# mpeg5/xevd

Measured on AMD Instinct MI355X. Metric: frames/sec (bit-exact YUV) + achieved HBM GB/s, higher is better.
Workload: dtype s16; 1 GPU; cfg4_main_8k_10b_ra; width=7680, height=4320, bit_depth=10, batches_resident=4, residual_pass_ahead=True, parallelism=1 stream on 1 GPU

## Files before the change

xevd_amd/csrc/itdq_body.h:

```cpp
#pragma once
#include "xgpu_internal.h"

typedef short v2s __attribute__((ext_vector_type(2)));

static __constant__ uint32_t k_tmp[2730];
__host__ __device__ constexpr int tmp_base(int log2n) { return log2n == 1 ? 0 : log2n == 2 ? 2 : log2n == 3 ? 10 : log2n == 4 ? 42 : log2n == 5 ? 170 : 682; }

static __constant__ uint32_t k_atsp[2][680];
__host__ __device__ constexpr int atsp_base(int log2n) { return log2n == 2 ? 0 : log2n == 3 ? 8 : log2n == 4 ? 40 : 168; }

static void upload_transform_tables_tu(const int *tm, const int16_t *ats, hipStream_t s)
{
    static uint32_t apk[2][680];
    for (int t = 0; t < 2; t++) {
        int src = 0;
        for (int l = 2; l <= 5; l++) {
            const int N = 1 << l, dst = atsp_base(l);
            for (int k2 = 0; k2 < N / 2; k2++)
                for (int n = 0; n < N; n++)
                    apk[t][dst + k2 * N + n] = (uint32_t)(uint16_t)ats[t * 1360 + src + (2 * k2) * N + n] |
                                               ((uint32_t)(uint16_t)ats[t * 1360 + src + (2 * k2 + 1) * N + n] << 16);
            src += N * N;
        }
    }
    (void)hipMemcpyToSymbolAsync(HIP_SYMBOL(k_atsp), apk, sizeof(apk), 0, hipMemcpyHostToDevice, s);
    static uint32_t packed[2730];
    int src = 0;
    for (int l = 1; l <= 6; l++) {
        const int N = 1 << l, dst = tmp_base(l);
        for (int k2 = 0; k2 < N / 2; k2++)
            for (int n = 0; n < N; n++)
                packed[dst + k2 * N + n] = (uint32_t)(uint16_t)(int16_t)tm[src + (2 * k2) * N + n] |
                                           ((uint32_t)(uint16_t)(int16_t)tm[src + (2 * k2 + 1) * N + n] << 16);
        src += N * N;
    }
    (void)hipMemcpyToSymbolAsync(HIP_SYMBOL(k_tmp), packed, sizeof(packed), 0, hipMemcpyHostToDevice, s);
    (void)hipStreamSynchronize(s);
}

__device__ __forceinline__ int clip16(int v) { return min(max(v, -32768), 32767); }
__device__ __forceinline__ int dot2(uint32_t a, uint32_t b, int c)
{
    return __builtin_amdgcn_sdot2(__builtin_bit_cast(v2s, a), __builtin_bit_cast(v2s, b), c, false);
}

__host__ __device__ constexpr int itdq_group(int lw, int lh)
{
    const int W = 1 << lw, H = 1 << lh;
    const int l1 = W * (H > 16 ? H / 16 : 1), l2 = H * (W > 16 ? W / 16 : 1);
    return 256 / (l1 > l2 ? l1 : l2);
}

#define ITDQ_PLANES_DWORDS 4608
#define ITDQ_LDS_DWORDS (ITDQ_PLANES_DWORDS + 2048)
#define ITDQ_MAX_G 128

__device__ __forceinline__ uint32_t wave_or(uint32_t v)
{
#pragma unroll
    for (int m = 32; m >= 1; m >>= 1) v |= (uint32_t)__shfl_xor((int)v, m, 64);
    return v;
}

template <int LW, int LH, bool IQT>
__device__ __forceinline__ void itdq_item(const ItdqArgs &a, const TbWave wv, uint32_t *lds, uint32_t *s_rm, uint32_t *s_cm)
{
    constexpr int W = 1 << LW, H = 1 << LH;
    constexpr int N1 = H > 16 ? 16 : H, C1 = H / N1;
    constexpr int N2 = W > 16 ? 16 : W, C2 = W / N2;
    constexpr int G = itdq_group(LW, LH);
    constexpr int RS = W / 2 + 1;
    constexpr int PLANE = G * H * RS;
    constexpr bool UNI1 = (G * W) % 64 == 0, UNI2 = (G * H) % 64 == 0;
    static_assert(2 * PLANE <= ITDQ_PLANES_DWORDS && G * W * H <= 4096 && G <= ITDQ_MAX_G, "LDS budget");
    constexpr int PLANES_DWORDS = IQT ? ITDQ_PLANES_DWORDS / 2 : ITDQ_PLANES_DWORDS;
    constexpr bool RMASK = H >= 16, CMASK = W >= 16;
    const int t = threadIdx.x;
    if (RMASK || CMASK) {
        if (t < G) { s_rm[t] = 0; s_cm[t] = 0; }
        __syncthreads();
    }
    const uint32_t *tmh = (wv.tr_v == TR_DCT2 || LH < 2 || LH > 5) ? k_tmp + tmp_base(LH) : k_atsp[wv.tr_v - 1] + atsp_base(LH);
    const uint32_t *tmw = (wv.tr_h == TR_DCT2 || LW < 2 || LW > 5) ? k_tmp + tmp_base(LW) : k_atsp[wv.tr_h - 1] + atsp_base(LW);
    const bool s16_mid = IQT || wv.tr_v != TR_DCT2 || wv.tr_h != TR_DCT2;
    int16_t *ldsh = (int16_t *)lds;
    int16_t *ldsl = (int16_t *)(lds + PLANE);
    uint32_t *ldsc = lds + PLANES_DWORDS;

    {
        constexpr int S = W * H, UN = S >= 8 ? 8 : 4;
        constexpr int odd = (LW + LH) & 1;
        const int shift = 20 - 14 - (15 - a.bd - ((LW + LH) >> 1)) + (odd ? 8 : 0);
        const long long offset = shift == 0 ? 0 : 1ll << (shift - 1);
        for (int u = t; u < G * S / UN; u += 256) {
            const int p = (u * UN) / S, o = (u * UN) % S;
            if (p >= wv.count) break;
            const TbRec tb = a.tbs[wv.first + p];
            const int qp = tb.qp, sidx = qp % 6;
            const int sbase = sidx == 0 ? 40 : sidx == 1 ? 45 : sidx == 2 ? 51 : sidx == 3 ? 57 : sidx == 4 ? 64 : (IQT ? 72 : 71);
            const long long mul = (long long)(sbase << (qp / 6)) * (odd ? 181 : 1);
            const int16_t *src = a.coef + tb.off + ((o >> LW) << tb.log2s) + (o & (W - 1));
            uint32_t raw[UN / 2];
            if constexpr (UN == 8) { const uint4 v = *(const uint4 *)src; raw[0] = v.x; raw[1] = v.y; raw[2] = v.z; raw[3] = v.w; }
            else { const uint2 v = *(const uint2 *)src; raw[0] = v.x; raw[1] = v.y; }
#pragma unroll
            for (int i = 0; i < UN / 2; i++) {
                if (raw[i] == 0) continue;
                const int c0 = (int16_t)(raw[i] & 0xFFFF), c1 = (int16_t)(raw[i] >> 16);
                const long long l0 = ((long long)c0 * mul + offset) >> shift, l1 = ((long long)c1 * mul + offset) >> shift;
                const int v0 = (int)min(max(l0, -32768ll), 32767ll), v1 = (int)min(max(l1, -32768ll), 32767ll);
                raw[i] = (uint32_t)(uint16_t)v0 | ((uint32_t)(uint16_t)v1 << 16);
                if (RMASK) atomicOr(&s_rm[p], 1u << ((o + 2 * i) >> (LW + 1)));
                if (CMASK) atomicOr(&s_cm[p], 1u << (((o + 2 * i) & (W - 1)) >> 1));
            }
#pragma unroll
            for (int i = 0; i < UN / 2; i++) ldsc[(p * S + o) / 2 + i] = raw[i];
        }
    }
    __syncthreads();

    uint32_t rows1 = 0;
    if (RMASK) {
        const int p1 = (t % (G * W)) >> LW;
        rows1 = (uint32_t)__builtin_amdgcn_readfirstlane((int)wave_or((t < G * W * C1 && p1 < wv.count) ? s_rm[p1] : 0u));
    }
    if (t < G * W * C1) {
        const int idx = t % (G * W);
        int chunk = t / (G * W);
        if (UNI1) chunk = __builtin_amdgcn_readfirstlane(chunk);
        const int p = idx >> LW, j = idx & (W - 1);
        const bool valid = p < wv.count;
        const int16_t *src = (const int16_t *)ldsc + p * (W * H) + j;

        int acc[N1];
#pragma unroll
        for (int n = 0; n < N1; n++) acc[n] = 0;
        if (RMASK) {
            for (uint32_t m = rows1; m; m &= m - 1) {
                const int k2 = __builtin_ctz(m);
                const uint32_t vp = valid ? ((uint32_t)(uint16_t)src[(2 * k2) * W] | ((uint32_t)(uint16_t)src[(2 * k2 + 1) * W] << 16)) : 0u;
                const uint32_t *row = tmh + k2 * H + chunk * N1;
#pragma unroll
                for (int n = 0; n < N1; n++) acc[n] = dot2(row[n], vp, acc[n]);
            }
        } else {
            for (int k2 = 0; k2 < H / 2; k2++) {
                const uint32_t vp = valid ? ((uint32_t)(uint16_t)src[(2 * k2) * W] | ((uint32_t)(uint16_t)src[(2 * k2 + 1) * W] << 16)) : 0u;
                if (__ballot(vp != 0) == 0) continue;
                const uint32_t *row = tmh + k2 * H + chunk * N1;
#pragma unroll
                for (int n = 0; n < N1; n++) acc[n] = dot2(row[n], vp, acc[n]);
            }
        }
        const int base = (p * H + chunk * N1) * (2 * RS) + j;
        if (CMASK && !(valid && ((s_cm[p] >> (j >> 1)) & 1))) {
        } else if (s16_mid) {
#pragma unroll
            for (int n = 0; n < N1; n++) ldsh[base + n * (2 * RS)] = (int16_t)clip16((acc[n] + 64) >> 7);
        } else {
#pragma unroll
            for (int n = 0; n < N1; n++) {
                ldsh[base + n * (2 * RS)] = (int16_t)(acc[n] >> 15);
                ldsl[base + n * (2 * RS)] = (int16_t)(acc[n] & 0x7FFF);
            }
        }
    }
    __syncthreads();

    uint32_t cols2 = 0;
    if (CMASK) {
        const int p2 = (t % (G * H)) >> LH;
        cols2 = (uint32_t)__builtin_amdgcn_readfirstlane((int)wave_or((t < G * H * C2 && p2 < wv.count) ? s_cm[p2] : 0u));
    }
    if (t < G * H * C2) {
        const int idx = t % (G * H);
        int chunk = t / (G * H);
        if (UNI2) chunk = __builtin_amdgcn_readfirstlane(chunk);
        const int p = idx >> LH, r = idx & (H - 1);
        if (p >= wv.count) return;
        const uint32_t own = CMASK ? s_cm[p] : 0xFFFFFFFFu;
        const TbRec tb = a.tbs[wv.first + p];
        const int shift2 = s16_mid ? 12 - (a.bd - 8) : 7 + 12 - (a.bd - 8);
        const uint32_t *inh = lds + (p * H + r) * RS;
        const uint32_t *inl = inh + PLANE;
        int res[N2];
        if (s16_mid) {
            int s[N2];
#pragma unroll
            for (int n = 0; n < N2; n++) s[n] = 1 << (shift2 - 1);
            if (CMASK) {
                for (uint32_t m = cols2; m; m &= m - 1) {
                    const int k2 = __builtin_ctz(m);
                    const uint32_t vp = ((own >> k2) & 1) ? inh[k2] : 0u;
                    const uint32_t *row = tmw + k2 * W + chunk * N2;
#pragma unroll
                    for (int n = 0; n < N2; n++) s[n] = dot2(row[n], vp, s[n]);
                }
            } else {
                for (int k2 = 0; k2 < W / 2; k2++) {
                    const uint32_t vp = inh[k2];
                    if (__ballot(vp != 0) == 0) continue;
                    const uint32_t *row = tmw + k2 * W + chunk * N2;
#pragma unroll
                    for (int n = 0; n < N2; n++) s[n] = dot2(row[n], vp, s[n]);
                }
            }
#pragma unroll
            for (int n = 0; n < N2; n++) res[n] = clip16(s[n] >> shift2);
        } else {
            int sh[N2], sl[N2];
#pragma unroll
            for (int n = 0; n < N2; n++) { sh[n] = 0; sl[n] = 0; }
            if (CMASK) {
                for (uint32_t m = cols2; m; m &= m - 1) {
                    const int k2 = __builtin_ctz(m);
                    const bool mine = (own >> k2) & 1;
                    const uint32_t vh = mine ? inh[k2] : 0u, vl = mine ? inl[k2] : 0u;
                    const uint32_t *row = tmw + k2 * W + chunk * N2;
#pragma unroll
                    for (int n = 0; n < N2; n++) { sh[n] = dot2(row[n], vh, sh[n]); sl[n] = dot2(row[n], vl, sl[n]); }
                }
            } else {
                for (int k2 = 0; k2 < W / 2; k2++) {
                    const uint32_t vh = inh[k2], vl = inl[k2];
                    if (__ballot((vh | vl) != 0) == 0) continue;
                    const uint32_t *row = tmw + k2 * W + chunk * N2;
#pragma unroll
                    for (int n = 0; n < N2; n++) { sh[n] = dot2(row[n], vh, sh[n]); sl[n] = dot2(row[n], vl, sl[n]); }
                }
            }
            const long long add = 1ll << (shift2 - 1);
#pragma unroll
            for (int n = 0; n < N2; n++) {
                const long long s = (long long)sh[n] * 32768 + sl[n] + add;
                res[n] = (int)min(max(s >> shift2, -32768ll), 32767ll);
            }
        }
        int16_t *out = a.resid + tb.off + (r << tb.log2s) + chunk * N2;
        if constexpr (N2 >= 8) {
#pragma unroll
            for (int n = 0; n < N2; n += 8) {
                uint4 v;
                v.x = (uint32_t)(uint16_t)res[n + 0] | ((uint32_t)(uint16_t)res[n + 1] << 16);
                v.y = (uint32_t)(uint16_t)res[n + 2] | ((uint32_t)(uint16_t)res[n + 3] << 16);
                v.z = (uint32_t)(uint16_t)res[n + 4] | ((uint32_t)(uint16_t)res[n + 5] << 16);
                v.w = (uint32_t)(uint16_t)res[n + 6] | ((uint32_t)(uint16_t)res[n + 7] << 16);
                *(uint4 *)(out + n) = v;
            }
        } else if constexpr (N2 == 4) {
            uint2 v;
            v.x = (uint32_t)(uint16_t)res[0] | ((uint32_t)(uint16_t)res[1] << 16);
            v.y = (uint32_t)(uint16_t)res[2] | ((uint32_t)(uint16_t)res[3] << 16);
            *(uint2 *)out = v;
        } else {
            *(uint32_t *)out = (uint32_t)(uint16_t)res[0] | ((uint32_t)(uint16_t)res[1] << 16);
        }
    }
}

template <bool IQT>
__device__ __forceinline__ void itdq_dispatch(const ItdqArgs &a, int wi, uint32_t *lds, uint32_t *s_rm, uint32_t *s_cm)
{
    const TbWave wv = a.waves[wi];
#define CASE(lw, lh) case (lw) * 8 + (lh): itdq_item<lw, lh, IQT>(a, wv, lds, s_rm, s_cm); break;
#define ROW(lw) CASE(lw, 1) CASE(lw, 2) CASE(lw, 3) CASE(lw, 4) CASE(lw, 5) CASE(lw, 6)
    switch (wv.log2w * 8 + wv.log2h) {
        ROW(1) ROW(2) ROW(3) ROW(4) ROW(5) ROW(6)
        default: break;
    }
#undef ROW
#undef CASE
}
```

xevd_amd/csrc/k_intra.hip:

```cpp
#include "xgpu_internal.h"
#include "itdq_body.h"

#include <type_traits>
#include "intra_pred.h"

#define INTRA_WAVES 8


__constant__ uint8_t k_htdf_tbl[5][16] = {
    { 0, 0, 2,  6, 10, 14, 19, 23, 28, 32,  36,  41,  45,  49,  53,  57 },
    { 0, 0, 5, 12, 20, 29, 38, 47, 56, 65,  73,  82,  90,  98, 107, 115 },
    { 0, 0, 1,  4,  9, 16, 24, 32, 41, 50,  59,  68,  77,  86,  94, 103 },
    { 0, 0, 3,  9, 19, 32, 47, 64, 81, 99, 117, 135, 154, 179, 205, 230 },
    { 0, 0, 0,  2,  6, 11, 18, 27, 38, 51,  64,  96, 128, 160, 192, 224 },
};
#define HTDF_EXT (66 * 66)

template <bool HTDF> struct IntraLds { static constexpr int WAVE = (HTDF && HTDF_EXT > 3 * NB_LEN) ? HTDF_EXT : 3 * NB_LEN; };

#ifdef INTRA_PROFILE
__device__ uint32_t g_intra_prof[8 * 64];
#define ISTAMP(k) do { if (DEP && t == 0 && item >= INTRA_PROFILE && item < INTRA_PROFILE + 64) g_intra_prof[8 * (item - INTRA_PROFILE) + (k)] = (uint32_t)clock64(); } while (0)
#else
#define ISTAMP(k)
// ... 315 lines not shown
                        for (int q = 0; q < 4; q++) pl[r][q] = vl[nb_sel(md, r, q, 3)];
                if (md == mode_c)
#pragma unroll
                    for (int c = 0; c < 2; c++)
#pragma unroll
                        for (int r = 0; r < 2; r++)
#pragma unroll
                            for (int q = 0; q < 2; q++) pc[c][r][q] = vc[c][nb_sel(md, r, q, 1)];
            }
            }
            int16_t *dy = a.cur_y + y * a.s_l + x;
            uint32_t ol[4][2], oc[2][2];
#pragma unroll
            for (int r = 0; r < 4; r++) {
                ol[r][0] = pack2i(pl[r][0], pl[r][1]); ol[r][1] = pack2i(pl[r][2], pl[r][3]);
                ol[r][0] = recon2i(ol[r][0], (cbf & 1) ? rl_cur[r].x : 0u, maxv); ol[r][1] = recon2i(ol[r][1], (cbf & 1) ? rl_cur[r].y : 0u, maxv);
            }
#pragma unroll
            for (int c = 1; c < 3; c++)
#pragma unroll
                for (int r = 0; r < 2; r++) {
                    oc[c - 1][r] = pack2i(pc[c - 1][r][0], pc[c - 1][r][1]);
                    oc[c - 1][r] = recon2i(oc[c - 1][r], ((cbf >> c) & 1) ? rc_cur[c - 1][r] : 0u, maxv);
                }
            const int coff = (y >> 1) * a.s_c + (x >> 1);
            if (!(nflags & 32u))
#pragma unroll
            for (int r = 0; r < 4; r++) {
                if (DEP) st_coherent2(dy + r * a.s_l, ol[r][0], ol[r][1]); else *(uint2 *)(dy + r * a.s_l) = make_uint2(ol[r][0], ol[r][1]);
            }
            if (!(nflags & 64u))
#pragma unroll
            for (int c = 1; c < 3; c++) {
                int16_t *d = (c == 1 ? a.cur_u : a.cur_v) + coff;
#pragma unroll
                for (int r = 0; r < 2; r++)
                    if (DEP) st_coherent(d + r * a.s_c, oc[c - 1][r]); else *(uint32_t *)(d + r * a.s_c) = oc[c - 1][r];
            }
        }
        if (HTDF && htdf_cu) {
            const uint32_t av = (nflags >> 8) & 0x1FF;
            const bool cmask = (nflags >> 4) & 1;
            const int tidx = (nflags >> 20) & 7;
            const int thr_log2 = tidx == 0 ? 6 : (tidx < 3 ? 7 : 8), shift = thr_log2 - 4, rnd = (1 << shift) >> 1, thr = (1 << thr_log2) - (1 << shift);
            int16_t *tb = s_nb[wv];
            wave_lds_sync();
            const int we = cw + 2, he = chh + 2;
            int16_t *org = a.cur_y + cu_y * a.s_l + cu_x;
            asm volatile("s_waitcnt vmcnt(0)" ::: "memory");
            auto ldw = [&](const int16_t *p) -> uint32_t { return DEP ? ld_coherent(p) : *(const uint32_t *)p; };
            auto ldr = [&](const int16_t *p) -> uint32_t { return ldw((const int16_t *)((uintptr_t)p & ~(uintptr_t)3)); };
            auto pick = [&](const int16_t *p, uint32_t d) -> int16_t { return (int16_t)(((uintptr_t)p & 2) ? d >> 16 : d & 0xFFFFu); };
            const int16_t *p_l = nullptr, *p_r = nullptr, *p_u = nullptr, *p_d = nullptr, *p_c = nullptr;
            uint32_t d_l = 0, d_r = 0, d_u = 0, d_d = 0, d_c = 0;
            if (t < chh) {
                const bool ok_l = ((av >> 1) & 1) && (!cmask || ((avail_le_raw >> (t >> 2)) & 1));
                const bool ok_r = ((av >> 3) & 1) && (!cmask || ((avail_ri >> (t >> 2)) & 1));
                p_l = org + t * a.s_l + (ok_l ? -1 : 0); p_r = org + t * a.s_l + (ok_r ? cw : cw - 1);
                d_l = ldr(p_l); d_r = ldr(p_r);
            }
            if (t < cw) {
                const bool ok_u = (av & 1) && (!cmask || ((avail_up >> (t >> 2)) & 1));
                p_u = org + t - (ok_u ? a.s_l : 0); p_d = org + (chh - 1) * a.s_l + t;
                d_u = ldr(p_u); d_d = ldr(p_d);
            }
            if (t < 4) {
                p_c = t == 0 ? (((av >> 5) & 1) ? org - 1 - a.s_l : org) : t == 1 ? (((av >> 6) & 1) ? org + cw - a.s_l : org + cw - 1)
                    : t == 2 ? (((av >> 7) & 1) ? org - 1 + chh * a.s_l : org + (chh - 1) * a.s_l) : (((av >> 8) & 1) ? org + cw + chh * a.s_l : org + cw - 1 + (chh - 1) * a.s_l);
                d_c = ldr(p_c);
            }
            const int n2 = (cw >> 1) * chh;
            ISTAMP(6);
            for (int i0 = 0; i0 < n2; i0 += 64 * 8) {
                uint32_t d[8];
#pragma unroll
                for (int q = 0; q < 8; q++) {
                    const int i = i0 + q * 64 + t;
                    d[q] = 0;
                    if (i < n2) d[q] = ldw(org + (i >> (lw - 1)) * a.s_l + ((i & ((cw >> 1) - 1)) << 1));
                }
#pragma unroll
                for (int q = 0; q < 8; q++) {
                    const int i = i0 + q * 64 + t, r = i >> (lw - 1), c = (i & ((cw >> 1) - 1)) << 1;
                    if (i < n2) { tb[(r + 1) * we + c + 1] = (int16_t)(d[q] & 0xFFFF); tb[(r + 1) * we + c + 2] = (int16_t)(d[q] >> 16); }
                }
            }
            asm volatile("" : "+v"(d_l), "+v"(d_r), "+v"(d_u), "+v"(d_d), "+v"(d_c));
            if (t < chh) { tb[(t + 1) * we] = pick(p_l, d_l); tb[(t + 1) * we + we - 1] = pick(p_r, d_r); }
            if (t < cw) { tb[t + 1] = pick(p_u, d_u); tb[(he - 1) * we + t + 1] = pick(p_d, d_d); }
            if (t < 4) tb[t == 0 ? 0 : t == 1 ? we - 1 : t == 2 ? we * (he - 1) : we - 1 + we * (he - 1)] = pick(p_c, d_c);
            wave_lds_sync();
            ISTAMP(7);
            const uint32_t *tb32 = (const uint32_t *)k_htdf_tbl[tidx];
            const uint32_t tq0 = uni(tb32[0]), tq1 = uni(tb32[1]), tq2 = uni(tb32[2]), tq3 = uni(tb32[3]);
            auto lutf = [&](int z) -> int {
                const int ab = z < 0 ? -z : z;
                const uint32_t idx = (uint32_t)(((ab + rnd) & thr) >> shift), sel = (idx & 7u) | 0x0C0C0C00u;
                const int e = (int)((idx & 8u) ? __builtin_amdgcn_perm(tq3, tq2, sel) : __builtin_amdgcn_perm(tq1, tq0, sel));
                const int v = ab < thr ? e : ab;
                return z < 0 ? -v : v;
            };
            auto filter_tiles = [&](auto TRc, auto TCc) {
                constexpr int TR = decltype(TRc)::value, TC = decltype(TCc)::value, LR = TR == 4 ? 2 : 1, LC = TC == 4 ? 2 : 1;
                const int tiles_x = cw >> LC, ltx = lw - LC;
                for (int i = t; i < tiles_x * (chh >> LR); i += 64) {
                    const int r = (i >> ltx) << LR, c = (i & (tiles_x - 1)) << LC;
                    int p[TR + 2][TC + 2];
#pragma unroll
                    for (int rr = 0; rr < TR + 2; rr++)
#pragma unroll
                        for (int cc = 0; cc < TC + 2; cc += 2) {
                            const uint32_t d = *(const uint32_t *)&tb[(r + rr) * we + c + cc];
                            p[rr][cc] = (int)(int16_t)(d & 0xFFFF); p[rr][cc + 1] = (int)(int16_t)(d >> 16);
                        }
                    int acc[TR][TC];
#pragma unroll
                    for (int dr = 0; dr < TR; dr++)
#pragma unroll
                        for (int dc = 0; dc < TC; dc++) acc[dr][dc] = 0;
#pragma unroll
                    for (int wr = 0; wr < TR + 1; wr++)
#pragma unroll
                        for (int wc = 0; wc < TC + 1; wc++) {
                            const int x0 = p[wr][wc], x1 = p[wr][wc + 1], x2 = p[wr + 1][wc], x3 = p[wr + 1][wc + 1];
                            const int y0 = x0 + x2, y1 = x1 + x3, y2 = x0 - x2, y3 = x1 - x3;
                            const int z0 = y0 + y1, z1 = lutf(y0 - y1), z2 = lutf(y2 + y3), z3 = lutf(y2 - y3);
                            const int i0_ = z0 + z2, i1_ = z1 + z3, i2_ = z0 - z2, i3_ = z1 - z3;
#pragma unroll
                            for (int row = 0; row < 2; row++)
#pragma unroll
                                for (int col = 0; col < 2; col++) {
                                    const int dr = wr - 1 + row, dc = wc - 1 + col;
                                    if (dr < 0 || dr >= TR || dc < 0 || dc >= TC) continue;
                                    const int v = row == 1 ? (col == 0 ? i2_ + i3_ : i2_ - i3_) : (col == 0 ? i0_ + i1_ : i0_ - i1_);
                                    acc[dr][dc] += v >> 2;
                                }
                        }
#pragma unroll
                    for (int dr = 0; dr < TR; dr++)
#pragma unroll
                        for (int dc = 0; dc < TC; dc += 2) {
                            const int o0 = clip3i(0, maxv, ((int)(int16_t)acc[dr][dc] + 2) >> 2), o1 = clip3i(0, maxv, ((int)(int16_t)acc[dr][dc + 1] + 2) >> 2);
                            if (DEP) st_coherent(org + (r + dr) * a.s_l + c + dc, pack2i(o0, o1)); else *(uint32_t *)(org + (r + dr) * a.s_l + c + dc) = pack2i(o0, o1);
                        }
                }
            };
            if (cw * chh >= 1024) filter_tiles(std::integral_constant<int, 4>{}, std::integral_constant<int, 4>{});
            else                 filter_tiles(std::integral_constant<int, 2>{}, std::integral_constant<int, 2>{});
        }
        ISTAMP(4);
        if (DEP) {
            asm volatile("s_waitcnt vmcnt(0)" ::: "memory");
            ISTAMP(5);
            if (t == 0) __hip_atomic_store(&a.done[item], a.epoch, __ATOMIC_RELAXED, __HIP_MEMORY_SCOPE_AGENT);
        }
        wave_lds_sync();
        if (!DEP) break;
        item = uni(q0.x);
        if (item == 0xFFFFFFFFu) break;
    }
}

#define SB_C0 71
#define SB_UR 144
#define SB_LEN (SB_UR + 72)
#define SMALL_GROUPS (4 * INTRA_WAVES)
__device__ __forceinline__ void intra_small_body(const IntraArgs &a, uint32_t block, int16_t *s_nb_)
{
    int16_t (*s_nb)[3][SB_LEN] = (int16_t (*)[3][SB_LEN])s_nb_;
    const int g = threadIdx.x >> 4, t = threadIdx.x & 15;
    const uint32_t k = block * SMALL_GROUPS + (uint32_t)g;
    if (k >= (uint32_t)a.n_small) return;
    const uint32_t item = (uint32_t)(a.first + a.count - a.n_small) + k;
    int16_t (*nb)[SB_LEN] = s_nb[g];
    const int mid = 1 << (a.bd_l - 1), maxv = (1 << a.bd_l) - 1;
    const uint4 *rec = (const uint4 *)&a.list[item];
    const uint4 q0 = rec[0], q1 = rec[1], q2 = rec[2];
    const uint32_t nflags = q0.y, avail_ul = nflags & 1;
    const int lrf = (int)((nflags >> 23) & 3);
    const uint64_t avail_up = (uint64_t)q0.z | ((lrf & 2) ? 0ull : (uint64_t)q0.w << 32);
    const uint64_t avail_le = (uint64_t)q1.x | ((uint64_t)q1.y << 32);
    const uint32_t gg = q2.x, m = q2.y, ipm = q2.z, coef_off = q2.w;
    const int cu_x = gg & 0xFFFF, cu_y = gg >> 16;
    const int lw = m & 0xFF, lh = (m >> 8) & 0xFF, cbf = (m >> 16) & 0xFF;
    const int mode_l = ipm & 0xFF, mode_c = (ipm >> 8) & 0xFF;
    const int cw = 1 << lw, chh = 1 << lh, scuw = cw >> 2, nscu = scuw * (chh >> 2), cwc = cw >> 1;
    const uint32_t off_u = coef_off + ((cbf & 1) ? (uint32_t)(cw * chh) : 0u);
    const uint32_t off_v = off_u + ((cbf & 2) ? (uint32_t)(cwc * (chh >> 1)) : 0u);
    const bool has = t < nscu;
    const int lx = (t & (scuw - 1)) << 2, ly = (t >> (lw - 2)) << 2;

    uint2 rl[4] = { { 0, 0 }, { 0, 0 }, { 0, 0 }, { 0, 0 } };
    uint32_t rc[2][2] = { { 0, 0 }, { 0, 0 } };
    if (has) {
        if (cbf & 1)
#pragma unroll
            for (int r = 0; r < 4; r++) rl[r] = *(const uint2 *)(a.resid + coef_off + (ly + r) * cw + lx);
#pragma unroll
        for (int c = 1; c < 3; c++)
            if ((cbf >> c) & 1)
#pragma unroll
                for (int r = 0; r < 2; r++) rc[c - 1][r] = *(const uint32_t *)(a.resid + (c == 1 ? off_u : off_v) + ((ly >> 1) + r) * cwc + (lx >> 1));
    }

#pragma unroll
    for (int c = 0; c < 3; c++) {
        const int16_t *plane = c == 0 ? a.cur_y : (c == 1 ? a.cur_u : a.cur_v);
        const int s = c ? a.s_c : a.s_l, sh = c ? 1 : 0, ush = c ? 1 : 2;
        const int16_t *org = plane + (cu_y >> sh) * s + (cu_x >> sh);
        const int n = (cw + chh) >> sh;
        const int eu = min(2 * t, n - 2), e0 = min(t, n - 1), e1 = min(t + 16, n - 1);
        const uint32_t vu = *(const uint32_t *)(org - s + eu);
        const uint32_t v0 = (uint16_t)org[e0 * s - 1], v1 = (uint16_t)org[e1 * s - 1], vc = (uint16_t)org[-s - 1];
        const uint32_t midp = (uint32_t)mid * 0x10001u;
        if (2 * t < n) *(uint32_t *)&nb[c][SB_C0 + 1 + 2 * t] = ((avail_up >> (eu >> ush)) & 1) ? vu : midp;
        if (t < n) nb[c][SB_C0 - 1 - t] = (int16_t)(((avail_le >> (e0 >> ush)) & 1) ? v0 : (uint32_t)mid);
        if (t + 16 < n) nb[c][SB_C0 - 1 - (t + 16)] = (int16_t)(((avail_le >> (e1 >> ush)) & 1) ? v1 : (uint32_t)mid);
        if (t == 0) nb[c][SB_C0] = (int16_t)(avail_ul ? vc : (uint32_t)mid);
        if (n > 32) {
            for (int e = 2 * t + 32; e < n; e += 32)
                *(uint32_t *)&nb[c][SB_C0 + 1 + e] = ((avail_up >> (e >> ush)) & 1) ? *(const uint32_t *)(org - s + e) : midp;
            for (int e = t + 32; e < n; e += 16)
                nb[c][SB_C0 - 1 - e] = ((avail_le >> (e >> ush)) & 1) ? org[e * s - 1] : (int16_t)mid;
        }
    }
    wave_lds_sync();
#pragma unroll
    for (int c = 0; c < 3; c++) {
        const int mode = c ? mode_c : mode_l;
        const int w = c ? cw >> 1 : cw, h = c ? chh >> 1 : chh;
        if (mode == 0) {
            int acc = 0;
            for (int e = t; e < w + h; e += 16) acc += e < h ? nb[c][SB_C0 - 1 - e] : nb[c][SB_C0 + 1 + e - h];
            acc = row_sum16(acc);
            if (t == 0) nb[c][NB_DC] = (int16_t)((acc + w) >> ((c ? lw - 1 : lw) + 1));
        } else if (mode == 4) {
            for (int e = t; e < w + h; e += 16) nb[c][SB_UR + e] = (int16_t)((nb[c][SB_C0 + 1 + e] + nb[c][SB_C0 - 1 - e]) >> 1);
        }
    }
    wave_lds_sync();
    if (!has) return;
    const int x = cu_x + lx, y = cu_y + ly;
    int pl[4][4], pc[2][2][2];
    int vl[7], vc[2][3];
    nb_fetch<7, SB_C0, SB_UR>(nb[0], mode_l, lx, ly, vl);
    nb_fetch<3, SB_C0, SB_UR>(nb[1], mode_c, lx >> 1, ly >> 1, vc[0]);
    nb_fetch<3, SB_C0, SB_UR>(nb[2], mode_c, lx >> 1, ly >> 1, vc[1]);
#pragma unroll
    for (int md = 0; md < 5; md++) {
        if (md == mode_l)
#pragma unroll
            for (int r = 0; r < 4; r++)
#pragma unroll
                for (int q = 0; q < 4; q++) pl[r][q] = vl[nb_sel(md, r, q, 3)];
        if (md == mode_c)
#pragma unroll
            for (int c = 0; c < 2; c++)
#pragma unroll
                for (int r = 0; r < 2; r++)
#pragma unroll
                    for (int q = 0; q < 2; q++) pc[c][r][q] = vc[c][nb_sel(md, r, q, 1)];
    }
    int16_t *dy = a.cur_y + y * a.s_l + x;
    const int coff = (y >> 1) * a.s_c + (x >> 1);
    if (!(nflags & 32u))
#pragma unroll
        for (int r = 0; r < 4; r++) {
            const uint32_t o0 = recon2i(pack2i(pl[r][0], pl[r][1]), (cbf & 1) ? rl[r].x : 0u, maxv), o1 = recon2i(pack2i(pl[r][2], pl[r][3]), (cbf & 1) ? rl[r].y : 0u, maxv);
            *(uint2 *)(dy + r * a.s_l) = make_uint2(o0, o1);
        }
    if (!(nflags & 64u))
#pragma unroll
        for (int c = 1; c < 3; c++) {
            int16_t *d = (c == 1 ? a.cur_u : a.cur_v) + coff;
#pragma unroll
            for (int r = 0; r < 2; r++)
                *(uint32_t *)(d + r * a.s_c) = recon2i(pack2i(pc[c - 1][r][0], pc[c - 1][r][1]), ((cbf >> c) & 1) ? rc[c - 1][r] : 0u, maxv);
        }
}

__global__ __launch_bounds__(64 * INTRA_WAVES) void k_intra_l1(const IntraArgs a, uint32_t big)
{
    constexpr int BIG_LDS = INTRA_WAVES * IntraLds<false>::WAVE, SMALL_LDS = SMALL_GROUPS * 3 * SB_LEN;
    __shared__ __attribute__((aligned(16))) int16_t s_nb[BIG_LDS > SMALL_LDS ? BIG_LDS : SMALL_LDS];
    if (blockIdx.x < big) {
        IntraArgs b = a;
        b.count = a.count - a.n_small;
        intra_body<false, 0, false, false, INTRA_WAVES>(b, blockIdx.x, s_nb, nullptr);
    } else intra_small_body(a, blockIdx.x - big, s_nb);
}

template <bool DEP, int EIPD, bool IBC, bool HTDF>
__global__ __launch_bounds__(64 * INTRA_WAVES) void k_intra(const IntraArgs a)
{
    __shared__ __attribute__((aligned(16))) int16_t s_nb[INTRA_WAVES * IntraLds<HTDF>::WAVE];
    __shared__ uint32_t s_chunk;
    intra_body<DEP, EIPD, IBC, HTDF, INTRA_WAVES>(a, blockIdx.x, s_nb, &s_chunk);
}

#define FUSED_WAVES 4
template <int EIPD, bool IBC, bool IQT>
__global__ __launch_bounds__(64 * FUSED_WAVES) void k_intra_itdq(const IntraArgs a, const ItdqArgs r, uint32_t n_intra_wg, uint64_t rate)
{
    constexpr int ITDQ_DW = (IQT ? ITDQ_LDS_DWORDS - ITDQ_PLANES_DWORDS / 2 : ITDQ_LDS_DWORDS) + 2 * ITDQ_MAX_G, INTRA_DW = (FUSED_WAVES * IntraLds<false>::WAVE + 1) / 2 + 4;
    __shared__ __attribute__((aligned(16))) uint32_t raw[ITDQ_DW > INTRA_DW ? ITDQ_DW : INTRA_DW];
    const uint32_t before = min(n_intra_wg, (uint32_t)(((uint64_t)blockIdx.x * rate) >> 32)), after = min(n_intra_wg, (uint32_t)(((uint64_t)(blockIdx.x + 1) * rate) >> 32));
    if (after > before) {
        intra_body<true, EIPD, IBC, false, FUSED_WAVES>(a, blockIdx.x, (int16_t *)raw, raw + INTRA_DW - 1);
    } else {
        const int wi = (int)(blockIdx.x - before);
        if (wi >= r.n_waves) return;
        uint32_t *s_rm = raw + ITDQ_DW - 2 * ITDQ_MAX_G;
        itdq_dispatch<IQT>(r, wi, raw, s_rm, s_rm + ITDQ_MAX_G);
    }
}

void upload_transform_tables_intra(const int *tm, const int16_t *ats, hipStream_t s) { upload_transform_tables_tu(tm, ats, s); }

int intra_chunk(bool with_itdq) { return with_itdq ? FUSED_WAVES : INTRA_WAVES; }

void launch_intra(xgpu_ctx *c, const IntraArgs &a, bool dep, bool ibc, bool htdf, const ItdqArgs *next, bool right)
{
    right = right && c->sp.tool_eipd;
    if (next) {
        const uint32_t n_wg = (uint32_t)((a.count + FUSED_WAVES - 1) / FUSED_WAVES);
        const dim3 g(n_wg + (uint32_t)next->n_waves), b(64 * FUSED_WAVES);
        const uint32_t span = std::max(n_wg, g.x / 2);
        const uint64_t rate = (((uint64_t)n_wg << 32) + span - 1) / span;
#define LAUNCHF(E, I) do { if (next->iqt) hipLaunchKernelGGL((k_intra_itdq<E, I, true>), g, b, 0, c->stream, a, *next, n_wg, rate); else hipLaunchKernelGGL((k_intra_itdq<E, I, false>), g, b, 0, c->stream, a, *next, n_wg, rate); } while (0)
        if (right) LAUNCHF(2, true);
        else if (c->sp.tool_eipd) { if (ibc) LAUNCHF(1, true); else LAUNCHF(1, false); }
        else                 { if (ibc) LAUNCHF(0, true); else LAUNCHF(0, false); }
#undef LAUNCHF
        return;
    }
    const int per = INTRA_WAVES;
    if (!dep && !right && !htdf && !ibc && !c->sp.tool_eipd && a.n_small >= c->intra_small_min) {
        const uint32_t big = (uint32_t)((a.count - a.n_small + per - 1) / per), small_blocks = (uint32_t)((a.n_small + SMALL_GROUPS - 1) / SMALL_GROUPS);
        hipLaunchKernelGGL(k_intra_l1, dim3(big + small_blocks), dim3(64 * INTRA_WAVES), 0, c->stream, a, big);
        return;
    }
    const int blocks = (a.count + per - 1) / per;
    const dim3 g(blocks), b(64 * INTRA_WAVES);
#define LAUNCH(D, E, I, H) hipLaunchKernelGGL((k_intra<D, E, I, H>), g, b, 0, c->stream, a)
    if (right) { if (dep) LAUNCH(true, 2, true, true); else LAUNCH(false, 2, true, true); }
    else if (htdf) {
        if (c->sp.tool_eipd) { if (dep) LAUNCH(true, 1, true, true); else LAUNCH(false, 1, true, true); }
        else                 { if (dep) LAUNCH(true, 0, true, true); else LAUNCH(false, 0, true, true); }
    } else if (ibc) {
        if (c->sp.tool_eipd) { if (dep) LAUNCH(true, 1, true, false); else LAUNCH(false, 1, true, false); }
        else                 { if (dep) LAUNCH(true, 0, true, false); else LAUNCH(false, 0, true, false); }
    } else {
        if (c->sp.tool_eipd) { if (dep) LAUNCH(true, 1, false, false); else LAUNCH(false, 1, false, false); }
        else                 { if (dep) LAUNCH(true, 0, false, false); else LAUNCH(false, 0, false, false); }
    }
#undef LAUNCH
#ifdef INTRA_PROFILE
    static int shots = 0;
    if (dep && ++shots == 5) {
        hipStreamSynchronize(c->stream);
        uint32_t h[8 * 64];
        hipMemcpyFromSymbol(h, HIP_SYMBOL(g_intra_prof), sizeof(h));
        for (int i = 0; i < 64; i++)
            fprintf(stderr, "  pos %d start %10u  wait %6u stage %5u (EIPD luma: issue %5u, return %5u | HTDF: to the block loads %5u from stamp 3, block in LDS %5u) plan %5u predict %5u ack %5u\n", INTRA_PROFILE + i, h[8 * i], h[8 * i + 1] - h[8 * i],
                    h[8 * i + 2] - h[8 * i + 1], h[8 * i + 6] - h[8 * i + 1], h[8 * i + 7] - h[8 * i + 6], h[8 * i + 6] - h[8 * i + 3], h[8 * i + 7] - h[8 * i + 6], h[8 * i + 3] - h[8 * i + 2], h[8 * i + 4] - h[8 * i + 3], h[8 * i + 5] - h[8 * i + 4]);
    }
#endif
}
```

xevd_amd/csrc/k_itdq.hip:

```cpp
#include "itdq_body.h"

template <bool IQT>
__global__ __launch_bounds__(256) void k_itdq(const ItdqArgs a)
{
    __shared__ uint32_t lds[IQT ? ITDQ_LDS_DWORDS - ITDQ_PLANES_DWORDS / 2 : ITDQ_LDS_DWORDS];
    __shared__ uint32_t s_rm[ITDQ_MAX_G], s_cm[ITDQ_MAX_G];
    const int wi = blockIdx.x;
    if (wi >= a.n_waves) return;
    itdq_dispatch<IQT>(a, wi, lds, s_rm, s_cm);
}

int itdq_group_size(int lw, int lh) { return itdq_group(lw, lh); }

void upload_transform_tables_intra(const int *tm, const int16_t *ats, hipStream_t s);
void upload_transform_tables(const int *tm, const int16_t *ats, hipStream_t s)
{
    upload_transform_tables_tu(tm, ats, s);
    upload_transform_tables_intra(tm, ats, s);
}

void launch_itdq(xgpu_ctx *c, const ItdqArgs &a, hipStream_t s)
{
    if (a.n_waves <= 0) return;
    if (a.iqt) hipLaunchKernelGGL(k_itdq<true>, dim3(a.n_waves), dim3(256), 0, s, a);
    else       hipLaunchKernelGGL(k_itdq<false>, dim3(a.n_waves), dim3(256), 0, s, a);
}
```

Measured before the change: 3369 frames/s.

## Add register-only ITDQ path for tiny TBs and streamline dequant and TB record loads

Transform blocks of 16 samples or fewer are now handled one per lane entirely in registers, skipping LDS staging and barriers. For larger blocks, the TB records and coefficients are prefetched up front and the records are cached in LDS for the second pass. Dequantisation for even sizes uses a 24-bit multiply-add with a pre-clamp instead of 64-bit arithmetic. Wave masks are built from a few LDS reads instead of a shuffle reduction, and several selects become bitwise masks. The tiny-TB path adds register pressure and assumes contiguous coefficient layout, since it ignores log2s.

```diff
diff --git a/xevd_amd/csrc/itdq_body.h b/xevd_amd/csrc/itdq_body.h
--- a/xevd_amd/csrc/itdq_body.h
+++ b/xevd_amd/csrc/itdq_body.h
@@ -1,5 +1,6 @@
 #pragma once
 #include "xgpu_internal.h"
+#include <type_traits>
 
 typedef short v2s __attribute__((ext_vector_type(2)));
 
@@ -43,6 +44,13 @@
 {
     return __builtin_amdgcn_sdot2(__builtin_bit_cast(v2s, a), __builtin_bit_cast(v2s, b), c, false);
 }
+__device__ __forceinline__ int mad24(int a, int b, int c)
+{
+    int r;
+    asm("v_mad_i32_i24 %0, %1, %2, %3" : "=v"(r) : "v"(a), "v"(b), "v"(c));
+    return r;
+}
+__device__ __forceinline__ uint32_t pack16(int lo, int hi) { return (uint32_t)(uint16_t)lo | ((uint32_t)hi << 16); }
 
 __host__ __device__ constexpr int itdq_group(int lw, int lh)
 {
@@ -53,17 +61,157 @@
 
 #define ITDQ_PLANES_DWORDS 4608
 #define ITDQ_LDS_DWORDS (ITDQ_PLANES_DWORDS + 2048)
-#define ITDQ_MAX_G 128
-
-__device__ __forceinline__ uint32_t wave_or(uint32_t v)
-{
-#pragma unroll
-    for (int m = 32; m >= 1; m >>= 1) v |= (uint32_t)__shfl_xor((int)v, m, 64);
-    return v;
-}
+#define ITDQ_MAX_G 32
+#define ITDQ_TB_DWORDS (4 * ITDQ_MAX_G)
+
+typedef uint32_t itq_v2 __attribute__((ext_vector_type(2)));
+typedef uint32_t itq_v4 __attribute__((ext_vector_type(4)));
+typedef itq_v2 __attribute__((aligned(4))) itq_v2_u;
+typedef itq_v4 __attribute__((aligned(2))) itq_v4_u;
+typedef itq_v2 __attribute__((aligned(2))) itq_v2_s;
+template <typename T> __device__ __forceinline__ T itq_any() { T v; asm volatile("" : "=v"(v)); return v; }
+static_assert(sizeof(TbRec) == 8, "a TbRec is fetched as one 8-byte load: off | log2w, log2h, qp, log2s");
+__device__ __forceinline__ void itq_rec_if(itq_v2 &v, const TbRec *p, bool on) { if (on) v = *(const itq_v2_u *)p; }
+__device__ __forceinline__ int rec_qp(itq_v2 r) { return (int)((r.y >> 16) & 0xFF); }
+__device__ __forceinline__ int rec_log2s(itq_v2 r) { return (int)(r.y >> 24); }
+
+template <bool ODD, bool IQT>
+struct ItdqScale {
+    int mul, cmax, shift, offset;
+    __device__ __forceinline__ ItdqScale(int qp, int bd, int lwh)
+    {
+        shift = bd - 9 + (lwh >> 1) + (ODD ? 8 : 0);
+        offset = shift == 0 ? 0 : 1 << (shift - 1);
+        const int q6 = (int)(((uint32_t)qp * 171u) >> 10), sidx = qp - 6 * q6;
+        constexpr uint64_t scale = 40ull | 45ull << 8 | 51ull << 16 | 57ull << 24 | 64ull << 32 | (uint64_t)(IQT ? 72 : 71) << 40;
+        const int sbase = (int)((scale >> (8 * sidx)) & 0xFF);
+        mul = sbase << q6;
+        cmax = (1 << 23) >> q6;
+    }
+    __device__ __forceinline__ int operator()(int c) const
+    {
+        if constexpr (!ODD) {
+            const int held = min(max(c, -cmax), cmax);
+            return clip16(mad24(held, mul, offset) >> shift);
+        }
+        const long long l = ((long long)(c * (ODD ? 181 : 1)) * mul + offset) >> shift;
+        return (int)min(max(l, -32768ll), 32767ll);
+    }
+};
+
+template <int G, int LX>
+__device__ __forceinline__ uint32_t wave_masks(const uint32_t *s_m, int t)
+{
+    constexpr int X = 1 << LX, PER = 64 / X > 1 ? 64 / X : 1, N = G < PER ? G : PER;
+    const int p0 = __builtin_amdgcn_readfirstlane(((t & ~63) % (G * X)) >> LX);
+    static_assert(G * X >= 64 ? (G % N == 0) : (64 % (G * X) == 0 && N == G), "the wave's TBs are entries [p0, p0 + N)");
+    uint32_t m = 0;
+#pragma unroll
+    for (int i = 0; i < N; i++) m |= s_m[p0 + i];
+    return (uint32_t)__builtin_amdgcn_readfirstlane((int)m);
+}
+
+template <int L>
+__device__ __forceinline__ const uint32_t *itdq_matrix(int tr) { return (tr == TR_DCT2 || L < 2 || L > 5) ? k_tmp + tmp_base(L) : k_atsp[tr - 1] + atsp_base(L); }
 
 template <int LW, int LH, bool IQT>
-__device__ __forceinline__ void itdq_item(const ItdqArgs &a, const TbWave wv, uint32_t *lds, uint32_t *s_rm, uint32_t *s_cm)
+__device__ __forceinline__ void itdq_small(const ItdqArgs &a, const TbWave wv)
+{
+    constexpr int W = 1 << LW, H = 1 << LH, S = W * H;
+    static_assert(S <= 16 && itdq_group(LW, LH) <= 256, "one TB per lane");
+    const int p = threadIdx.x;
+    if (p >= wv.count) return;
+    const itq_v2 rec = *(const itq_v2_u *)(a.tbs + wv.first + p);
+    const uint32_t *tmh = itdq_matrix<LH>(wv.tr_v), *tmw = itdq_matrix<LW>(wv.tr_h);
+    const bool s16_mid = IQT || wv.tr_v != TR_DCT2 || wv.tr_h != TR_DCT2;
+    uint32_t raw[S / 2];
+    if constexpr (S == 4) { const itq_v2 v = *(const itq_v2_s *)(a.coef + rec.x); raw[0] = v.x; raw[1] = v.y; }
+    else {
+#pragma unroll
+        for (int i = 0; i < S / 8; i++) {
+            const itq_v4 v = *(const itq_v4_u *)(a.coef + rec.x + 8 * i);
+            raw[4 * i] = v.x; raw[4 * i + 1] = v.y; raw[4 * i + 2] = v.z; raw[4 * i + 3] = v.w;
+        }
+    }
+    const ItdqScale<(LW + LH) & 1, IQT> dq(rec_qp(rec), a.bd, LW + LH);
+    int d[S];
+#pragma unroll
+    for (int i = 0; i < S / 2; i++) {
+        d[2 * i] = 0; d[2 * i + 1] = 0;
+        if (raw[i] != 0) { d[2 * i] = dq((int16_t)(raw[i] & 0xFFFF)); d[2 * i + 1] = dq((int16_t)(raw[i] >> 16)); }
+    }
+    uint32_t mh[H][W / 2], ml[H][W / 2];
+#pragma unroll
+    for (int jj = 0; jj < W / 2; jj++) {
+        int acc[2][H];
+#pragma unroll
+        for (int e = 0; e < 2; e++) {
+#pragma unroll
+            for (int n = 0; n < H; n++) acc[e][n] = 0;
+#pragma unroll
+            for (int k2 = 0; k2 < H / 2; k2++) {
+                const uint32_t vp = pack16(d[(2 * k2) * W + 2 * jj + e], d[(2 * k2 + 1) * W + 2 * jj + e]);
+#pragma unroll
+                for (int n = 0; n < H; n++) acc[e][n] = dot2(tmh[k2 * H + n], vp, acc[e][n]);
+            }
+        }
+#pragma unroll
+        for (int n = 0; n < H; n++) {
+            if (s16_mid) mh[n][jj] = pack16(clip16((acc[0][n] + 64) >> 7), clip16((acc[1][n] + 64) >> 7));
+            else if constexpr (!IQT) {
+                mh[n][jj] = pack16(acc[0][n] >> 15, acc[1][n] >> 15);
+                ml[n][jj] = pack16(acc[0][n] & 0x7FFF, acc[1][n] & 0x7FFF);
+            }
+        }
+    }
+    const int shift2 = s16_mid ? 12 - (a.bd - 8) : 7 + 12 - (a.bd - 8);
+    uint32_t out[S / 2];
+#pragma unroll
+    for (int r = 0; r < H; r++) {
+        int res[W];
+        if (s16_mid) {
+            int s[W];
+#pragma unroll
+            for (int n = 0; n < W; n++) s[n] = 1 << (shift2 - 1);
+#pragma unroll
+            for (int k2 = 0; k2 < W / 2; k2++) {
+#pragma unroll
+                for (int n = 0; n < W; n++) s[n] = dot2(tmw[k2 * W + n], mh[r][k2], s[n]);
+            }
+#pragma unroll
+            for (int n = 0; n < W; n++) res[n] = clip16(s[n] >> shift2);
+        } else if constexpr (!IQT) {
+            int sh[W], sl[W];
+#pragma unroll
+            for (int n = 0; n < W; n++) { sh[n] = 0; sl[n] = 0; }
+#pragma unroll
+            for (int k2 = 0; k2 < W / 2; k2++) {
+#pragma unroll
+                for (int n = 0; n < W; n++) { sh[n] = dot2(tmw[k2 * W + n], mh[r][k2], sh[n]); sl[n] = dot2(tmw[k2 * W + n], ml[r][k2], sl[n]); }
+            }
+            const long long add = 1ll << (shift2 - 1);
+#pragma unroll
+            for (int n = 0; n < W; n++) {
+                const long long s = (long long)sh[n] * 32768 + sl[n] + add;
+                res[n] = (int)min(max(s >> shift2, -32768ll), 32767ll);
+            }
+        }
+#pragma unroll
+        for (int n = 0; n < W; n += 2) out[(r * W + n) / 2] = pack16(res[n], res[n + 1]);
+    }
+    int16_t *dst = a.resid + rec.x;
+    if constexpr (S == 4) { itq_v2 v; v.x = out[0]; v.y = out[1]; *(itq_v2_s *)dst = v; }
+    else {
+#pragma unroll
+        for (int i = 0; i < S / 8; i++) {
+            itq_v4 v; v.x = out[4 * i]; v.y = out[4 * i + 1]; v.z = out[4 * i + 2]; v.w = out[4 * i + 3];
+            *(itq_v4_u *)(dst + 8 * i) = v;
+        }
+    }
+}
+
+template <int LW, int LH, bool IQT>
+__device__ __forceinline__ void itdq_item(const ItdqArgs &a, const TbWave wv, uint32_t *lds, uint32_t *s_tb)
 {
     constexpr int W = 1 << LW, H = 1 << LH;
     constexpr int N1 = H > 16 ? 16 : H, C1 = H / N1;
@@ -75,61 +223,71 @@
     static_assert(2 * PLANE <= ITDQ_PLANES_DWORDS && G * W * H <= 4096 && G <= ITDQ_MAX_G, "LDS budget");
     constexpr int PLANES_DWORDS = IQT ? ITDQ_PLANES_DWORDS / 2 : ITDQ_PLANES_DWORDS;
     constexpr bool RMASK = H >= 16, CMASK = W >= 16;
+    uint32_t *s_rm = s_tb, *s_cm = s_tb + ITDQ_MAX_G, *s_rec = s_tb + 2 * ITDQ_MAX_G;
     const int t = threadIdx.x;
+
+    constexpr int S = W * H, UN = S >= 8 ? 8 : 4, NU = G * S / UN, NR = (NU + 255) / 256;
+    typedef typename std::conditional<UN == 8, itq_v4, itq_v2>::type cvec;
+    bool on[NR];
+    int up[NR], uo[NR];
+    itq_v2 rec[NR];
+#pragma unroll
+    for (int r = 0; r < NR; r++) {
+        const int u = t + 256 * r;
+        up[r] = (u * UN) / S; uo[r] = (u * UN) % S;
+        on[r] = (NU % 256 == 0 || u < NU) && up[r] < wv.count;
+        rec[r] = itq_any<itq_v2>();
+        itq_rec_if(rec[r], a.tbs + wv.first + up[r], on[r]);
+    }
     if (RMASK || CMASK) {
         if (t < G) { s_rm[t] = 0; s_cm[t] = 0; }
         __syncthreads();
     }
-    const uint32_t *tmh = (wv.tr_v == TR_DCT2 || LH < 2 || LH > 5) ? k_tmp + tmp_base(LH) : k_atsp[wv.tr_v - 1] + atsp_base(LH);
-    const uint32_t *tmw = (wv.tr_h == TR_DCT2 || LW < 2 || LW > 5) ? k_tmp + tmp_base(LW) : k_atsp[wv.tr_h - 1] + atsp_base(LW);
+    const uint32_t *tmh = itdq_matrix<LH>(wv.tr_v), *tmw = itdq_matrix<LW>(wv.tr_h);
     const bool s16_mid = IQT || wv.tr_v != TR_DCT2 || wv.tr_h != TR_DCT2;
+    asm volatile("" :: "s"(tmh), "s"(tmw));
     int16_t *ldsh = (int16_t *)lds;
     int16_t *ldsl = (int16_t *)(lds + PLANE);
     uint32_t *ldsc = lds + PLANES_DWORDS;
-
-    {
-        constexpr int S = W * H, UN = S >= 8 ? 8 : 4;
-        constexpr int odd = (LW + LH) & 1;
-        const int shift = 20 - 14 - (15 - a.bd - ((LW + LH) >> 1)) + (odd ? 8 : 0);
-        const long long offset = shift == 0 ? 0 : 1ll << (shift - 1);
-        for (int u = t; u < G * S / UN; u += 256) {
-            const int p = (u * UN) / S, o = (u * UN) % S;
-            if (p >= wv.count) break;
-            const TbRec tb = a.tbs[wv.first + p];
-            const int qp = tb.qp, sidx = qp % 6;
-            const int sbase = sidx == 0 ? 40 : sidx == 1 ? 45 : sidx == 2 ? 51 : sidx == 3 ? 57 : sidx == 4 ? 64 : (IQT ? 72 : 71);
-            const long long mul = (long long)(sbase << (qp / 6)) * (odd ? 181 : 1);
-            const int16_t *src = a.coef + tb.off + ((o >> LW) << tb.log2s) + (o & (W - 1));
-            uint32_t raw[UN / 2];
-            if constexpr (UN == 8) { const uint4 v = *(const uint4 *)src; raw[0] = v.x; raw[1] = v.y; raw[2] = v.z; raw[3] = v.w; }
-            else { const uint2 v = *(const uint2 *)src; raw[0] = v.x; raw[1] = v.y; }
-#pragma unroll
-            for (int i = 0; i < UN / 2; i++) {
-                if (raw[i] == 0) continue;
-                const int c0 = (int16_t)(raw[i] & 0xFFFF), c1 = (int16_t)(raw[i] >> 16);
-                const long long l0 = ((long long)c0 * mul + offset) >> shift, l1 = ((long long)c1 * mul + offset) >> shift;
-                const int v0 = (int)min(max(l0, -32768ll), 32767ll), v1 = (int)min(max(l1, -32768ll), 32767ll);
-                raw[i] = (uint32_t)(uint16_t)v0 | ((uint32_t)(uint16_t)v1 << 16);
-                if (RMASK) atomicOr(&s_rm[p], 1u << ((o + 2 * i) >> (LW + 1)));
-                if (CMASK) atomicOr(&s_cm[p], 1u << (((o + 2 * i) & (W - 1)) >> 1));
-            }
-#pragma unroll
-            for (int i = 0; i < UN / 2; i++) ldsc[(p * S + o) / 2 + i] = raw[i];
-        }
+    cvec cv[NR];
+#pragma unroll
+    for (int r = 0; r < NR; r++) {
+        cv[r] = itq_any<cvec>();
+        if (on[r]) {
+            const int16_t *src = a.coef + rec[r].x + ((uo[r] >> LW) << rec_log2s(rec[r])) + (uo[r] & (W - 1));
+            if constexpr (UN == 8) cv[r] = *(const itq_v4_u *)src; else cv[r] = *(const itq_v2_s *)src;
+        }
+    }
+#pragma unroll
+    for (int r = 0; r < NR; r++) {
+        if (!on[r]) continue;
+        const int p = up[r], o = uo[r];
+        const ItdqScale<(LW + LH) & 1, IQT> dq(rec_qp(rec[r]), a.bd, LW + LH);
+        if (o == 0) { s_rec[2 * p] = rec[r].x; s_rec[2 * p + 1] = rec[r].y; }
+        uint32_t raw[UN / 2];
+#pragma unroll
+        for (int i = 0; i < UN / 2; i++) raw[i] = cv[r][i];
+#pragma unroll
+        for (int i = 0; i < UN / 2; i++) {
+            if (raw[i] == 0) continue;
+            raw[i] = pack16(dq((int16_t)(raw[i] & 0xFFFF)), dq((int16_t)(raw[i] >> 16)));
+            if (RMASK) atomicOr(&s_rm[p], 1u << ((o + 2 * i) >> (LW + 1)));
+            if (CMASK) atomicOr(&s_cm[p], 1u << (((o + 2 * i) & (W - 1)) >> 1));
+        }
+#pragma unroll
+        for (int i = 0; i < UN / 2; i++) ldsc[(p * S + o) / 2 + i] = raw[i];
     }
     __syncthreads();
 
     uint32_t rows1 = 0;
-    if (RMASK) {
-        const int p1 = (t % (G * W)) >> LW;
-        rows1 = (uint32_t)__builtin_amdgcn_readfirstlane((int)wave_or((t < G * W * C1 && p1 < wv.count) ? s_rm[p1] : 0u));
-    }
+    if (RMASK) rows1 = wave_masks<G, LW>(s_rm, t);
     if (t < G * W * C1) {
         const int idx = t % (G * W);
         int chunk = t / (G * W);
         if (UNI1) chunk = __builtin_amdgcn_readfirstlane(chunk);
         const int p = idx >> LW, j = idx & (W - 1);
         const bool valid = p < wv.count;
+        const uint32_t vmask = valid ? 0xFFFFFFFFu : 0u;
         const int16_t *src = (const int16_t *)ldsc + p * (W * H) + j;
 
         int acc[N1];
@@ -138,14 +296,14 @@
         if (RMASK) {
             for (uint32_t m = rows1; m; m &= m - 1) {
                 const int k2 = __builtin_ctz(m);
-                const uint32_t vp = valid ? ((uint32_t)(uint16_t)src[(2 * k2) * W] | ((uint32_t)(uint16_t)src[(2 * k2 + 1) * W] << 16)) : 0u;
+                const uint32_t vp = pack16(src[(2 * k2) * W], src[(2 * k2 + 1) * W]) & vmask;
                 const uint32_t *row = tmh + k2 * H + chunk * N1;
 #pragma unroll
                 for (int n = 0; n < N1; n++) acc[n] = dot2(row[n], vp, acc[n]);
             }
         } else {
             for (int k2 = 0; k2 < H / 2; k2++) {
-                const uint32_t vp = valid ? ((uint32_t)(uint16_t)src[(2 * k2) * W] | ((uint32_t)(uint16_t)src[(2 * k2 + 1) * W] << 16)) : 0u;
+                const uint32_t vp = pack16(src[(2 * k2) * W], src[(2 * k2 + 1) * W]) & vmask;
                 if (__ballot(vp != 0) == 0) continue;
                 const uint32_t *row = tmh + k2 * H + chunk * N1;
 #pragma unroll
@@ -168,10 +326,7 @@
     __syncthreads();
 
     uint32_t cols2 = 0;
-    if (CMASK) {
-        const int p2 = (t % (G * H)) >> LH;
-        cols2 = (uint32_t)__builtin_amdgcn_readfirstlane((int)wave_or((t < G * H * C2 && p2 < wv.count) ? s_cm[p2] : 0u));
-    }
+    if (CMASK) cols2 = wave_masks<G, LH>(s_cm, t);
     if (t < G * H * C2) {
         const int idx = t % (G * H);
         int chunk = t / (G * H);
@@ -179,7 +334,8 @@
         const int p = idx >> LH, r = idx & (H - 1);
         if (p >= wv.count) return;
         const uint32_t own = CMASK ? s_cm[p] : 0xFFFFFFFFu;
-        const TbRec tb = a.tbs[wv.first + p];
+        itq_v2 tb;
+        tb.x = s_rec[2 * p]; tb.y = s_rec[2 * p + 1];
         const int shift2 = s16_mid ? 12 - (a.bd - 8) : 7 + 12 - (a.bd - 8);
         const uint32_t *inh = lds + (p * H + r) * RS;
         const uint32_t *inl = inh + PLANE;
@@ -191,7 +347,7 @@
             if (CMASK) {
                 for (uint32_t m = cols2; m; m &= m - 1) {
                     const int k2 = __builtin_ctz(m);
-                    const uint32_t vp = ((own >> k2) & 1) ? inh[k2] : 0u;
+                    const uint32_t vp = inh[k2] & (0u - ((own >> k2) & 1));
                     const uint32_t *row = tmw + k2 * W + chunk * N2;
 #pragma unroll
                     for (int n = 0; n < N2; n++) s[n] = dot2(row[n], vp, s[n]);
@@ -214,8 +370,8 @@
             if (CMASK) {
                 for (uint32_t m = cols2; m; m &= m - 1) {
                     const int k2 = __builtin_ctz(m);
-                    const bool mine = (own >> k2) & 1;
-                    const uint32_t vh = mine ? inh[k2] : 0u, vl = mine ? inl[k2] : 0u;
+                    const uint32_t mine = 0u - ((own >> k2) & 1);
+                    const uint32_t vh = inh[k2] & mine, vl = inl[k2] & mine;
                     const uint32_t *row = tmw + k2 * W + chunk * N2;
 #pragma unroll
                     for (int n = 0; n < N2; n++) { sh[n] = dot2(row[n], vh, sh[n]); sl[n] = dot2(row[n], vl, sl[n]); }
@@ -236,33 +392,37 @@
                 res[n] = (int)min(max(s >> shift2, -32768ll), 32767ll);
             }
         }
-        int16_t *out = a.resid + tb.off + (r << tb.log2s) + chunk * N2;
+        int16_t *out = a.resid + tb.x + (r << rec_log2s(tb)) + chunk * N2;
         if constexpr (N2 >= 8) {
 #pragma unroll
             for (int n = 0; n < N2; n += 8) {
                 uint4 v;
-                v.x = (uint32_t)(uint16_t)res[n + 0] | ((uint32_t)(uint16_t)res[n + 1] << 16);
-                v.y = (uint32_t)(uint16_t)res[n + 2] | ((uint32_t)(uint16_t)res[n + 3] << 16);
-                v.z = (uint32_t)(uint16_t)res[n + 4] | ((uint32_t)(uint16_t)res[n + 5] << 16);
-                v.w = (uint32_t)(uint16_t)res[n + 6] | ((uint32_t)(uint16_t)res[n + 7] << 16);
+                v.x = pack16(res[n + 0], res[n + 1]);
+                v.y = pack16(res[n + 2], res[n + 3]);
+                v.z = pack16(res[n + 4], res[n + 5]);
+                v.w = pack16(res[n + 6], res[n + 7]);
                 *(uint4 *)(out + n) = v;
             }
         } else if constexpr (N2 == 4) {
             uint2 v;
-            v.x = (uint32_t)(uint16_t)res[0] | ((uint32_t)(uint16_t)res[1] << 16);
-            v.y = (uint32_t)(uint16_t)res[2] | ((uint32_t)(uint16_t)res[3] << 16);
+            v.x = pack16(res[0], res[1]);
+            v.y = pack16(res[2], res[3]);
             *(uint2 *)out = v;
         } else {
-            *(uint32_t *)out = (uint32_t)(uint16_t)res[0] | ((uint32_t)(uint16_t)res[1] << 16);
+            *(uint32_t *)out = pack16(res[0], res[1]);
         }
     }
 }
 
 template <bool IQT>
-__device__ __forceinline__ void itdq_dispatch(const ItdqArgs &a, int wi, uint32_t *lds, uint32_t *s_rm, uint32_t *s_cm)
-{
-    const TbWave wv = a.waves[wi];
-#define CASE(lw, lh) case (lw) * 8 + (lh): itdq_item<lw, lh, IQT>(a, wv, lds, s_rm, s_cm); break;
+__device__ __forceinline__ void itdq_dispatch(const ItdqArgs &a, int wi, uint32_t *lds, uint32_t *s_tb)
+{
+    static_assert(sizeof(TbWave) == 12 && alignof(TbWave) == 4, "TbWave is read as three dwords");
+    const uint32_t *w = (const uint32_t *)(a.waves + wi);
+    const uint32_t w0 = w[0], w1 = w[1], w2 = w[2];
+    TbWave wv;
+    wv.first = w0; wv.count = (uint16_t)(w1 & 0xFFFF); wv.log2w = (uint8_t)(w1 >> 16); wv.log2h = (uint8_t)(w1 >> 24); wv.tr_v = (uint8_t)w2; wv.tr_h = (uint8_t)(w2 >> 8);
+#define CASE(lw, lh) case (lw) * 8 + (lh): if constexpr ((lw) + (lh) <= 4) itdq_small<lw, lh, IQT>(a, wv); else itdq_item<lw, lh, IQT>(a, wv, lds, s_tb); break;
 #define ROW(lw) CASE(lw, 1) CASE(lw, 2) CASE(lw, 3) CASE(lw, 4) CASE(lw, 5) CASE(lw, 6)
     switch (wv.log2w * 8 + wv.log2h) {
         ROW(1) ROW(2) ROW(3) ROW(4) ROW(5) ROW(6)
diff --git a/xevd_amd/csrc/k_intra.hip b/xevd_amd/csrc/k_intra.hip
--- a/xevd_amd/csrc/k_intra.hip
+++ b/xevd_amd/csrc/k_intra.hip
@@ -641,7 +641,7 @@
 template <int EIPD, bool IBC, bool IQT>
 __global__ __launch_bounds__(64 * FUSED_WAVES) void k_intra_itdq(const IntraArgs a, const ItdqArgs r, uint32_t n_intra_wg, uint64_t rate)
 {
-    constexpr int ITDQ_DW = (IQT ? ITDQ_LDS_DWORDS - ITDQ_PLANES_DWORDS / 2 : ITDQ_LDS_DWORDS) + 2 * ITDQ_MAX_G, INTRA_DW = (FUSED_WAVES * IntraLds<false>::WAVE + 1) / 2 + 4;
+    constexpr int ITDQ_DW = (IQT ? ITDQ_LDS_DWORDS - ITDQ_PLANES_DWORDS / 2 : ITDQ_LDS_DWORDS) + ITDQ_TB_DWORDS, INTRA_DW = (FUSED_WAVES * IntraLds<false>::WAVE + 1) / 2 + 4;
     __shared__ __attribute__((aligned(16))) uint32_t raw[ITDQ_DW > INTRA_DW ? ITDQ_DW : INTRA_DW];
     const uint32_t before = min(n_intra_wg, (uint32_t)(((uint64_t)blockIdx.x * rate) >> 32)), after = min(n_intra_wg, (uint32_t)(((uint64_t)(blockIdx.x + 1) * rate) >> 32));
     if (after > before) {
@@ -649,8 +649,7 @@
     } else {
         const int wi = (int)(blockIdx.x - before);
         if (wi >= r.n_waves) return;
-        uint32_t *s_rm = raw + ITDQ_DW - 2 * ITDQ_MAX_G;
-        itdq_dispatch<IQT>(r, wi, raw, s_rm, s_rm + ITDQ_MAX_G);
+        itdq_dispatch<IQT>(r, wi, raw, raw + ITDQ_DW - ITDQ_TB_DWORDS);
     }
 }
 
diff --git a/xevd_amd/csrc/k_itdq.hip b/xevd_amd/csrc/k_itdq.hip
--- a/xevd_amd/csrc/k_itdq.hip
+++ b/xevd_amd/csrc/k_itdq.hip
@@ -4,10 +4,10 @@
 __global__ __launch_bounds__(256) void k_itdq(const ItdqArgs a)
 {
     __shared__ uint32_t lds[IQT ? ITDQ_LDS_DWORDS - ITDQ_PLANES_DWORDS / 2 : ITDQ_LDS_DWORDS];
-    __shared__ uint32_t s_rm[ITDQ_MAX_G], s_cm[ITDQ_MAX_G];
+    __shared__ uint32_t s_tb[ITDQ_TB_DWORDS];
     const int wi = blockIdx.x;
     if (wi >= a.n_waves) return;
-    itdq_dispatch<IQT>(a, wi, lds, s_rm, s_cm);
+    itdq_dispatch<IQT>(a, wi, lds, s_tb);
 }
 
 int itdq_group_size(int lw, int lh) { return itdq_group(lw, lh); }
```

Measured after the change: 3449 frames/s (median of 6 runs). 1.02x the previous value.
